# zhukovanadezhda/collaborative-filtering

Hardware: AMD Instinct MI355X
Metric: ratings/sec per ALS iteration at k=64 (higher is better)
Workload: dtype f32 (storage, solve, accumulate); Gram products as 2-way fp16 split (error <= 2^-23) on fp16 MFMA; rows over the condition limit redone in f64 (solve_dtype=auto)

## Files before the change

collaborative-filtering_amd/_hip.py:

```python
from __future__ import annotations

import ctypes as C
import os

_HERE = os.path.dirname(os.path.abspath(__file__))
LIB_PATH = os.environ.get("ALS_HIP_LIB") or os.path.join(_HERE, "csrc", "libals_hip.so")

SPLIT_CHUNK = 4096
MAX_K = 160

EXPORTS = ("als_version", "als_padded_k", "als_perm_index", "als_partial_slot_bytes", "als_partial_slot_bytes_f64",
           "als_row_solve", "als_factor_scale", "als_gs_sweep", "als_gs_sweep_levels", "als_gs_sweep_dataflow", "als_residual_stats", "als_w_normal_equations", "als_spd_solve_workspace_bytes", "als_spd_solve_f64", "als_item_stats", "als_item_stats_f64", "als_sum_pairs", "als_sumsq_partials",
           "als_sumsq", "als_history_row", "als_compose_z", "als_predict_at", "als_predict_dense",
           "als_topk_similarity", "als_graph_classify", "als_normalize_features", "als_impute_col_median",
           "als_host_coo_to_sides", "als_host_row_tasks", "als_host_level_schedule",
           "als_recommend_workspace_bytes", "als_recommend_topk", "als_rank_count_workspace_bytes", "als_rank_count",
           "als_recommend_topk_masked", "als_rank_count_masked",
           "als_fold_in", "als_fold_in_items", "als_explain", "als_mmr_rerank", "als_list_diversity")

_vp, _i32, _i64, _f32 = C.c_void_p, C.c_int32, C.c_int64, C.c_float


class RowSolveParams(C.Structure):
    _fields_ = [
        ("k", _i32), ("ld", _i32), ("nrows", _i64), ("F_zero_row", _i32), ("reserved0", _i32),
        ("gram_mode", _i32), ("ndual_tail", _i32), ("ndual_mid", _i32), ("F_scale_ready", _i32),
# ... 151 lines not shown
```

collaborative-filtering_amd/backend.py:

```python
from __future__ import annotations

import ctypes as C
import os
from typing import Optional

import torch

from . import _hip


def _p(t: Optional[torch.Tensor]):
    return None if t is None else C.c_void_p(t.data_ptr())


class HipBackend:
    name = "hip"

    GRAM_MODES = {"f32": 0, "f16x2": 1, "f64": 2}
    COND_LIMIT = 300.0
    PLANES_MAX_FLOATS = 16 << 20
    PLANES_MAX_FLOATS_K128 = (1 << 31) - 1

    def __init__(self, device: torch.device, gram: str = "f16x2", solve_dtype: str = "auto"):
        if gram not in ("f32", "f16x2"):
# ... 55 lines not shown
        p.sumr2_out, p.stat_out = _p(sumr2_out), _p(stat_out)
        p.tasks, p.ntasks = _p(tasks.tasks), tasks.ntasks
        p.ndual_tail = int(tasks.ndual)
        p.ndual_mid = int(tasks.nmid)
        p.long_rows, p.nlong = _p(tasks.long_rows), tasks.nlong
        p.workspace = _p(workspace)
        p.F_scale, p.F_scale_ready = _p(self._fscale), 0
        nwords = (int(zero_row) + 1) * ld
        limit = self.planes_max_floats if ld == 64 else (self.planes_max_floats_k128 if ld == 128 else 0)
        if (not f64 and p.gram_mode == self.GRAM_MODES["f16x2"] and 0 < nwords <= limit
                and int(zero_row) >= F.shape[0] - 1 and F.is_contiguous()):
            buf = self._planes.get(nwords)
            if buf is None:
                buf = self._planes[nwords] = torch.empty(nwords, dtype=torch.int32, device=self.device)
            p.F_planes = _p(buf)
        if self.cond_limit > 0.0 and not self.ablate and not f64:
            if side.nrows not in self._redo_rows:
                self._redo_rows[side.nrows] = torch.empty(max(side.nrows, 1), dtype=torch.int32, device=self.device)
            p.cond_limit = self.cond_limit
            p.redo_count, p.redo_rows = _p(self._redo_count), _p(self._redo_rows[side.nrows])
            p.cond_out = _p(self.cond_probe) if (self.cond_probe is not None and self.cond_probe.numel() >= side.nrows) else None
        self._check(self.lib.als_row_solve(C.byref(p), self._stream()), "als_row_solve")

    def gs_level(self, *, items, **kw):
        p = self._gs_params(items, kw)
        self._check(self.lib.als_gs_sweep(C.byref(p), self._stream()), "als_gs_sweep")

    def _gs_params(self, items, kw):
        p = _hip.GsSweepParams()
        p.k, p.ld = kw["k"], kw["ld"]
        p.items, p.nitems = _p(items), items.numel()
# ... 223 lines not shown
```

collaborative-filtering_amd/csrc/als_device.hpp:

```cpp
#pragma once
#include <hip/hip_runtime.h>
#include <stdint.h>
#include <type_traits>

typedef float f32x4 __attribute__((ext_vector_type(4)));
typedef float f32x2 __attribute__((ext_vector_type(2)));

#define ALS_EPS 1e-10f

#define ALS_KB_CASE_(N, ...) case N: { constexpr int KB = N; __VA_ARGS__; } break;
#define ALS_DISPATCH_KB(kb, ...)                                                                           \
    switch (kb) {                                                                                          \
        ALS_KB_CASE_(1, __VA_ARGS__) ALS_KB_CASE_(2, __VA_ARGS__) ALS_KB_CASE_(3, __VA_ARGS__)             \
        ALS_KB_CASE_(4, __VA_ARGS__) ALS_KB_CASE_(5, __VA_ARGS__) ALS_KB_CASE_(6, __VA_ARGS__)             \
        ALS_KB_CASE_(7, __VA_ARGS__) ALS_KB_CASE_(8, __VA_ARGS__) ALS_KB_CASE_(9, __VA_ARGS__)             \
        ALS_KB_CASE_(10, __VA_ARGS__)                                                                      \
        default: return ALS_E_BADK;                                                                        \
    }

__device__ __forceinline__ float readlane_f(float v, int src_lane) {
    return __int_as_float(__builtin_amdgcn_readlane(__float_as_int(v), src_lane));
}
__device__ __forceinline__ float bperm_f(float v, int src_lane) {
    return __int_as_float(__builtin_amdgcn_ds_bpermute(src_lane << 2, __float_as_int(v)));
}
__device__ __forceinline__ int bperm_i(int v, int src_lane) {
    return __builtin_amdgcn_ds_bpermute(src_lane << 2, v);
}
template <unsigned long long MASK>
__device__ __forceinline__ float select_lanes(float a, float b) {
    return __builtin_amdgcn_inverse_ballot_w64(MASK) ? a : b;
}
template <int BOUND, int RR>
constexpr unsigned long long lanes_below() {
    constexpr int n = BOUND - 64 * RR;
    return n <= 0 ? 0ull : (n >= 64 ? ~0ull : ((1ull << n) - 1ull));
}

__device__ __forceinline__ float wave_sum(float v) {
    auto dpp = [](float x, auto ctrl, auto rows) {
        return __int_as_float(__builtin_amdgcn_update_dpp(0, __float_as_int(x), decltype(ctrl)::value,
                                                          decltype(rows)::value, 0xf, false));
    };
    using std::integral_constant;
    v += dpp(v, integral_constant<int, 0xB1>{}, integral_constant<int, 0xf>{});
    v += dpp(v, integral_constant<int, 0x4E>{}, integral_constant<int, 0xf>{});
// ... 11 lines not shown
    uint32_t u = (uint32_t)__float_as_int(v);
    u = max(u, dpp(u, integral_constant<int, 0xB1>{}, integral_constant<int, 0xf>{}));
    u = max(u, dpp(u, integral_constant<int, 0x4E>{}, integral_constant<int, 0xf>{}));
    u = max(u, dpp(u, integral_constant<int, 0x141>{}, integral_constant<int, 0xf>{}));
    u = max(u, dpp(u, integral_constant<int, 0x140>{}, integral_constant<int, 0xf>{}));
    u = max(u, dpp(u, integral_constant<int, 0x142>{}, integral_constant<int, 0xa>{}));
    u = max(u, dpp(u, integral_constant<int, 0x143>{}, integral_constant<int, 0xc>{}));
    return __int_as_float(__builtin_amdgcn_readlane((int)u, 63));
}
__device__ __forceinline__ double wave_sum_d(double v) {
#pragma unroll
    for (int o = 32; o >= 1; o >>= 1) v += __shfl_xor(v, o, 64);
    return v;
}

__device__ __forceinline__ void wave_lds_sync() {
    __builtin_amdgcn_fence(__ATOMIC_SEQ_CST, "workgroup");
    __builtin_amdgcn_wave_barrier();
}

template <int KB>
__device__ __forceinline__ int perm_to_col(int p) { return KB * (p & 15) + (p >> 4); }

template <int KB>
__device__ __forceinline__ void load_frow(const float* __restrict__ p, float (&f)[KB]) {
    if constexpr (KB % 4 == 0) {
#pragma unroll
        for (int j = 0; j < KB / 4; ++j) {
            f32x4 v = *reinterpret_cast<const f32x4*>(p + 4 * j);
            f[4 * j] = v.x; f[4 * j + 1] = v.y; f[4 * j + 2] = v.z; f[4 * j + 3] = v.w;
        }
    } else if constexpr (KB % 2 == 0) {
// ... 400 lines not shown
```

collaborative-filtering_amd/csrc/row_common.hpp:

```cpp
#pragma once
#include <type_traits>
#include "als_device.hpp"

namespace {

__host__ __device__ constexpr int blk_idx(int I, int K) { return I * (I + 1) / 2 + K; }

typedef _Float16 h16x8 __attribute__((ext_vector_type(8)));
typedef _Float16 h16x2 __attribute__((ext_vector_type(2)));
typedef int i32x4 __attribute__((ext_vector_type(4)));

__device__ __forceinline__ void split2(float x0, float x1, float S, int& H, int& L) {
    const float y0 = x0 * S, y1 = x1 * S;
    const h16x2 h = __builtin_convertvector(f32x2{y0, y1}, h16x2);
    const float d0 = fmaf((float)h[0], -1.0f, y0), d1 = fmaf((float)h[1], -1.0f, y1);
    const h16x2 l = __builtin_convertvector(f32x2{d0, d1}, h16x2);
    H = __builtin_bit_cast(int, h);
    L = __builtin_bit_cast(int, l);
}

__device__ __forceinline__ void mfma_results_settle() {
    __builtin_amdgcn_sched_barrier(0);
    asm volatile("s_nop 15\n\ts_nop 3" ::: "memory");
    __builtin_amdgcn_sched_barrier(0);
}

template <int KB>
struct Chol {
    static constexpr int NR = KCfg<KB>::NR;
    float di[NR];
    float y[NR];
    float b[NR];
};

template <int KB>
__device__ __forceinline__ bool chol_spd(const Chol<KB>& S, int lane) {
    bool bad = false;
#pragma unroll
    for (int rr = 0; rr < KCfg<KB>::NR; ++rr) {
        const float v = S.di[rr];
        bad = bad || ((lane + 64 * rr < KCfg<KB>::KP) && !(v > 0.f && v < __builtin_inff()));
    }
    return __builtin_amdgcn_ballot_w64(bad) == 0;
}

template <int KB, int T2>
__device__ __forceinline__ void panel_trailing(float (&p)[KCfg<KB>::NR][16], const float (&l)[KCfg<KB>::NR], float lrep) {
    if constexpr (T2 < 16) {
#pragma unroll
        for (int rr = 0; rr < KCfg<KB>::NR; ++rr)
            asm("v_fmac_f32_dpp %0, %1, %2 row_newbcast:%3 row_mask:0xf bank_mask:0xf"
                : "+v"(p[rr][T2]) : "v"(lrep), "v"(l[rr]), "n"(T2));
        panel_trailing<KB, T2 + 1>(p, l, lrep);
    }
}

template <int KB, int RR, int T, int PB>
__device__ __forceinline__ void bwd_coeff_one(const float* __restrict__ Ls, const int (&colbase)[KCfg<KB>::NR][4],
                                              const Chol<KB>& S, float (&cf)[KCfg<KB>::NR][16]) {
    constexpr int prow = 16 * PB + T;
    const float v = Ls[colbase[RR][(T >> 2) & 3] + prow * 16];
    cf[RR][T] = select_lanes<lanes_below<prow, RR>()>(v * S.di[RR], 0.f);
    if constexpr (T + 1 < 16) bwd_coeff_one<KB, RR, T + 1, PB>(Ls, colbase, S, cf);
    else if constexpr (RR + 1 < KCfg<KB>::NR) bwd_coeff_one<KB, RR + 1, 0, PB>(Ls, colbase, S, cf);
}
template <int KB, int PB0>
__device__ __forceinline__ void bwd_coeffs(const float* __restrict__ Ls, const int (&colbase)[KCfg<KB>::NR][4],
                                           const Chol<KB>& S, float (&cf)[KCfg<KB>::NR][16],
                                           std::integral_constant<int, PB0>, int pb) {
    if (pb == PB0) bwd_coeff_one<KB, 0, 0, PB0>(Ls, colbase, S, cf);
    else if constexpr (PB0 + 1 < KB) bwd_coeffs<KB>(Ls, colbase, S, cf, std::integral_constant<int, PB0 + 1>{}, pb);
}

template <int KB>
__device__ __forceinline__ void backward_solve(const float* __restrict__ Ls, const Chol<KB>& S,
                                               float (&x)[KCfg<KB>::NR], int lane) {
    using C = KCfg<KB>;
// ... 31 lines not shown
```

collaborative-filtering_amd/csrc/row_solve.hip:

```cpp
#include <type_traits>
#include "als_device.hpp"
#include "als_hip.h"
#include "row_common.hpp"
#include "slot_fold.hpp"

namespace {

template <int KB>
struct RowAcc {
    f32x4 acc[KCfg<KB>::NACC];
    float rhs[KB];
    float cs[KB];
    float sumr;
    float sumr2;
    __device__ __forceinline__ void zero() {
#pragma unroll
        for (int a = 0; a < KCfg<KB>::NACC; ++a) acc[a] = f32x4{0.f, 0.f, 0.f, 0.f};
#pragma unroll
        for (int b = 0; b < KB; ++b) { rhs[b] = 0.f; cs[b] = 0.f; }
        sumr = 0.f; sumr2 = 0.f;
    }
};

template <int KB, bool FULL>
// ... 160 lines not shown
#pragma unroll
        for (int r = 0; r < 4; ++r) {
            Ls[(a * 4 + r) * 64 + lane] = A.acc[a][r];
            A.acc[a][r] = 0.f;
        }
}

template <int KB>
__device__ __forceinline__ void unflush_acc(RowAcc<KB>& A, const float* __restrict__ Ls, int lane) {
#pragma unroll
    for (int a = 0; a < KCfg<KB>::NACC; ++a)
#pragma unroll
        for (int r = 0; r < 4; ++r) A.acc[a][r] += Ls[(a * 4 + r) * 64 + lane];
}

template <int KB, int MODE>
__device__ __forceinline__ void gram_accumulate(RowAcc<KB>& A, const int32_t* __restrict__ idxp,
                                                const float* __restrict__ valp, int len,
                                                const float* __restrict__ F, int ld, int zero_row,
                                                const float* __restrict__ bias_other, float mu,
                                                float bself, int lane, float* __restrict__ Ls, float S,
                                                const uint32_t* __restrict__ planes = nullptr) {
    const int c = lane & 15, q = lane >> 4;
    const float* Fc = F + KB * c;
    int nflush = 0;
    f32x4 E[MODE == 2 ? KB : 1];
    const uint32_t* Pc = planes + KB * c;
    const int sel_c = (c == 0) ? 0x05040100 : (c == 2) ? 0x07060302 : 0x0c0c0c0c;
    const int ones_c = (c == 1) ? 0x3C003C00 : 0;
    const float inv_s = __int_as_float((254 - ((__float_as_int(S) >> 23) & 0xff)) << 23);
    if constexpr (MODE == 2) {
#pragma unroll
        for (int b = 0; b < KB; ++b) E[b] = f32x4{0.f, 0.f, 0.f, 0.f};
    }
    int idx1 = (lane < len) ? __builtin_nontemporal_load(idxp + lane) : zero_row;
    int idx2 = (64 + lane < len) ? __builtin_nontemporal_load(idxp + 64 + lane) : zero_row;
    float val1 = (lane < len) ? __builtin_nontemporal_load(valp + lane) : 0.f;
    float bo1 = (lane < len) ? bias_other[idx1] : 0.f;
    for (int base = 0; base < len; base += 64) {
        const int idx0 = idx1;
        const float val0 = val1, bo0 = bo1;
        idx1 = idx2;
        const int t2 = base + 128 + lane;
        idx2 = (t2 < len) ? __builtin_nontemporal_load(idxp + t2) : zero_row;
        const int t1 = base + 64 + lane;
        val1 = (t1 < len) ? __builtin_nontemporal_load(valp + t1) : 0.f;
        bo1 = (t1 < len) ? bias_other[idx1] : 0.f;
        const int nvalid = min(64, len - base);
        const bool ok = lane < nvalid;
        const float rb = val0 - mu - bo0;
        A.sumr += ok ? rb : 0.f;
        A.sumr2 = ok ? fmaf(rb, rb, A.sumr2) : A.sumr2;
        const float r0 = ok ? (rb - bself) : 0.f;
// ... 65 lines not shown
    constexpr int DR = (16 * J) >> 6, DL = (16 * J) & 63;
    const float prep = bperm_f(p[DR][T], DL + (lane & 15));
    const float d = readlane_f(p[RP][T], LP);
    const float inv = __builtin_amdgcn_rsqf(d);
    float l[NR];
#pragma unroll
    for (int rr = 0; rr < NR; ++rr) { l[rr] = p[rr][T] * inv; p[rr][T] = l[rr]; }
    float lrep = -(prep * inv);
    asm("s_nop 1" : "+v"(lrep));
    float yt = 0.f;
    if constexpr (SOLVE) yt = readlane_f(S.b[RP], LP) * inv;
    panel_trailing<KB, T + 1>(p, l, lrep);
    if constexpr (SOLVE) {
#pragma unroll
        for (int rr = 0; rr < NR; ++rr) S.b[rr] = fmaf(-l[rr], yt, S.b[rr]);
        S.y[RP] = select_lanes<1ull << LP>(yt, S.y[RP]);
    }
}

template <int KB, int J, int T, bool SOLVE>
__device__ __forceinline__ void panel_pivots(float (&p)[KCfg<KB>::NR][16], Chol<KB>& S, int lane) {
    if constexpr (T < 16) {
        panel_pivot<KB, J, T, SOLVE>(p, S, lane);
        panel_pivots<KB, J, T + 1, SOLVE>(p, S, lane);
    }
}

template <int KB, int J, bool SOLVE>
__device__ __forceinline__ void chol_panel(RowAcc<KB>& A, Chol<KB>& S, float* __restrict__ Ls, int lane) {
    using C = KCfg<KB>;
    constexpr int KP = C::KP, NR = C::NR;
    constexpr int OFF = C::lcol_off(J);
    const int c = lane & 15, q = lane >> 4;
    {
        const int swzc = (((c >> 2) ^ q) << 2) + (c & 3);
#pragma unroll
        for (int I = J; I < KB; ++I)
#pragma unroll
            for (int r = 0; r < 4; ++r)
                Ls[OFF + (16 * (I - J) + 4 * q + r) * 16 + swzc] = A.acc[blk_idx(I, J)][r];
    }
    wave_lds_sync();
    float p[NR][16];
    const int si = (lane >> 2) & 3;
#pragma unroll
    for (int rr = 0; rr < NR; ++rr) {
        const int i = lane + 64 * rr;
        const int rowi = min(max(i, 16 * J), KP - 1) - 16 * J;
#pragma unroll
        for (int g = 0; g < 4; ++g) {
            const f32x4 v = *reinterpret_cast<const f32x4*>(Ls + OFF + rowi * 16 + ((g ^ si) << 2));
            p[rr][4 * g] = v.x; p[rr][4 * g + 1] = v.y; p[rr][4 * g + 2] = v.z; p[rr][4 * g + 3] = v.w;
        }
    }
    wave_lds_sync();
    panel_pivots<KB, J, 0, SOLVE>(p, S, lane);
#pragma unroll
    for (int rr = 0; rr < NR; ++rr) {
        const int i = lane + 64 * rr;
        if (i >= 16 * J && i < KP) {
#pragma unroll
            for (int g = 0; g < 4; ++g) {
                const f32x4 v = {p[rr][4 * g], p[rr][4 * g + 1], p[rr][4 * g + 2], p[rr][4 * g + 3]};
                *reinterpret_cast<f32x4*>(Ls + OFF + (i - 16 * J) * 16 + ((g ^ si) << 2)) = v;
            }
        }
    }
    wave_lds_sync();
    {
        constexpr int DR = (16 * J) >> 6, DL = (16 * J) & 63;
        const float dl = Ls[OFF + c * 16 + (c & 3)];
        S.di[DR] = select_lanes<0xFFFFull << DL>(__builtin_amdgcn_rcpf(dl), S.di[DR]);
    }
    if constexpr (J + 1 < KB) {
        f32x4 op[KB - J - 1];
        const int sg = ((q ^ ((c >> 2) & 3)) << 2);
#pragma unroll
        for (int I = J + 1; I < KB; ++I)
            op[I - J - 1] = *reinterpret_cast<const f32x4*>(Ls + OFF + (16 * (I - J) + c) * 16 + sg);
#pragma unroll
        for (int K = J + 1; K < KB; ++K) {
            const f32x4 nb = -op[K - J - 1];
#pragma unroll
            for (int I = K; I < KB; ++I)
#pragma unroll
                for (int e = 0; e < 4; ++e)
                    A.acc[blk_idx(I, K)] = __builtin_amdgcn_mfma_f32_16x16x4f32(
                        op[I - J - 1][e], nb[e], A.acc[blk_idx(I, K)], 0, 0, 0);
        }
    }
}

template <int KB, int J, bool SOLVE>
__device__ __forceinline__ void chol_panels(RowAcc<KB>& A, Chol<KB>& S, float* __restrict__ Ls, int lane) {
    if constexpr (J < KB) {
        chol_panel<KB, J, SOLVE>(A, S, Ls, lane);
        chol_panels<KB, J + 1, SOLVE>(A, S, Ls, lane);
    }
}

template <int KB>
__device__ __forceinline__ bool row_needs_f64(const Chol<KB>& S, const als_row_solve_params& P, int row, bool spd,
                                              float mean_eig, float short_row_bound, int lane) {
    float dmx = 0.f, dmn = 0.f;
#pragma unroll
    for (int rr = 0; rr < KCfg<KB>::NR; ++rr) {
        const bool in = lane + 64 * rr < KCfg<KB>::KP;
        const float d = in ? S.di[rr] : 0.f;
        dmx = fmaxf(dmx, d);
        dmn = fmaxf(dmn, in ? __builtin_amdgcn_rcpf(d) : 0.f);
    }
    dmx = wave_max_nonneg(fmaxf(dmx, 0.f));
// ... 7 lines not shown
}

template <int KB>
__device__ __forceinline__ float gram_trace(const RowAcc<KB>& A, int lane) {
    const int c = lane & 15, q = lane >> 4;
    float t = 0.f;
#pragma unroll
    for (int J = 0; J < KB; ++J) {
        const f32x4 a = A.acc[blk_idx(J, J)];
        const float lo = (c & 1) ? a[1] : a[0], hi = (c & 1) ? a[3] : a[2];
        t += (c & 2) ? hi : lo;
    }
    return wave_sum((q == (c >> 2)) ? t : 0.f);
}

template <int KB>
__device__ __forceinline__ void finish_row(RowAcc<KB>& A, const als_row_solve_params& P, int row,
                                           float* __restrict__ Ls, int lane) {
    using C = KCfg<KB>;
    constexpr int KP = C::KP, NR = C::NR;
    const int c = lane & 15, q = lane >> 4;
    const int64_t r64 = row;

    if (P.gram_mode == ALS_GRAM_F16X2) {
        const float un = P.F_scale[1];
#pragma unroll
        for (int a = 0; a < C::NACC; ++a) A.acc[a] *= un;
    }

#pragma unroll
    for (int b = 0; b < KB; ++b) {
        A.rhs[b] += __shfl_xor(A.rhs[b], 16, 64); A.rhs[b] += __shfl_xor(A.rhs[b], 32, 64);
        A.cs[b] += __shfl_xor(A.cs[b], 16, 64);   A.cs[b] += __shfl_xor(A.cs[b], 32, 64);
    }
    const float sumr = wave_sum(A.sumr);
    const float sumr2 = wave_sum(A.sumr2);

    Chol<KB> S;
    float csrow[NR];
    int colrow[NR];
#pragma unroll
    for (int rr = 0; rr < NR; ++rr) {
        float bsel = 0.f, csel = 0.f;
#pragma unroll
        for (int e = 0; e < 4; ++e) {
            constexpr int dummy = 0; (void)dummy;
            const int b = (4 * rr + e < KB) ? 4 * rr + e : KB - 1;
            if (4 * rr + e < KB) {
                bsel = (q == e) ? A.rhs[b] : bsel;
                csel = (q == e) ? A.cs[b] : csel;
            }
        }
        S.b[rr] = bsel; S.di[rr] = 0.f; S.y[rr] = 0.f;
        csrow[rr] = csel;
        colrow[rr] = perm_to_col<KB>(min(lane + 64 * rr, KP - 1));
    }

    if (P.gram_out) {
        float* G = P.gram_out + r64 * KP * KP;
#pragma unroll
        for (int I = 0; I < KB; ++I)
#pragma unroll
            for (int K = 0; K <= I; ++K)
#pragma unroll
                for (int r = 0; r < 4; ++r)
                    G[(16 * I + 4 * q + r) * KP + 16 * K + c] = A.acc[blk_idx(I, K)][r];
    }
#pragma unroll
    for (int rr = 0; rr < NR; ++rr) {
        const int i = lane + 64 * rr;
        if (i < KP) {
            if (P.rhs_out) P.rhs_out[r64 * KP + i] = S.b[rr];
            if (P.colsum_out) P.colsum_out[r64 * KP + i] = csrow[rr];
        }
    }
    if (P.sumr_out && lane == 0) P.sumr_out[row] = sumr;
    if (P.sumr2_out && lane == 0) P.sumr2_out[row] = sumr2;

    const float lam = (P.lambda_row ? P.lambda_row[row] : P.lambda_scalar) + ALS_EPS
                    + (P.diag_extra ? P.diag_extra[row] : 0.f);
    float mean_eig = 0.f, short_row_bound = 0.f;
    if (P.cond_limit > 0.f) {
        const int64_t nrat = P.indptr[row + 1] - P.indptr[row];
        mean_eig = gram_trace<KB>(A, lane) / fmaxf((float)min((int64_t)P.k, nrat), 1.f) + lam;
        short_row_bound = (nrat < 4 * (int64_t)P.k) ? mean_eig / lam : 0.f;
    }
#pragma unroll
    for (int J = 0; J < KB; ++J) {
        const float dv = (perm_to_col<KB>(16 * J + c) < P.k) ? lam : 1.0f;
#pragma unroll
        for (int r = 0; r < 4; ++r) A.acc[blk_idx(J, J)][r] += (4 * q + r == c) ? dv : 0.f;
    }

    if (P.factor_out) {
        chol_panels<KB, 0, false>(A, S, Ls, lane);
        const bool spd = chol_spd<KB>(S, lane);
        if (P.cond_limit > 0.f) {
            if (row_needs_f64<KB>(S, P, row, spd, mean_eig, short_row_bound, lane)) return;
        } else if (!spd && lane == 0) atomicMax(P.status, row + 1);
        float* M = P.factor_out + r64 * KP * KP;
#pragma unroll
        for (int rr = 0; rr < NR; ++rr) {
            const int i = lane + 64 * rr;
            const int ic = min(i, KP - 1);
            const int colb = C::lcol_off_rt(ic >> 4) - 16 * (ic >> 4) * 16 + (c & 3);
#pragma unroll 8
            for (int p = 0; p < KP; ++p) {
                const int Jp = p >> 4;
                const int rowv = max(ic, 16 * Jp);
                const float lrow = Ls[C::lcol_off_rt(Jp) + (rowv - 16 * Jp) * 16 +
                                      ((((p >> 2) & 3) ^ ((rowv >> 2) & 3)) << 2) + (p & 3)];
                const int rsafe = max(p, ic & ~15);
                const float lcolv = Ls[colb + rsafe * 16 + (((c >> 2) ^ ((rsafe >> 2) & 3)) << 2)];
                if (i < KP) __builtin_nontemporal_store((p == i) ? S.di[rr] : (p < i ? lrow : lcolv), M + p * KP + i);
            }
        }
        return;
    }

    float rhs0[NR];
#pragma unroll
    for (int rr = 0; rr < NR; ++rr) rhs0[rr] = S.b[rr];
    if (P.rhs_extra) {
#pragma unroll
        for (int rr = 0; rr < NR; ++rr)
            if (lane + 64 * rr < KP) S.b[rr] += P.rhs_extra[r64 * P.ld + colrow[rr]];
    }
    if (!(P.reserved0 & 2)) {
        chol_panels<KB, 0, true>(A, S, Ls, lane);
        const bool spd = chol_spd<KB>(S, lane);
        if (P.cond_limit > 0.f) {
            if (row_needs_f64<KB>(S, P, row, spd, mean_eig, short_row_bound, lane)) return;
        } else if (!spd && lane == 0) atomicMax(P.status, row + 1);
    }
    float x[NR];
    if (!(P.reserved0 & 4)) backward_solve<KB>(Ls, S, x, lane);
    else {
#pragma unroll
        for (int rr = 0; rr < NR; ++rr) x[rr] = S.y[rr];
    }

    float dot = 0.f, xr = 0.f, yy = 0.f, xx = 0.f;
#pragma unroll
    for (int rr = 0; rr < NR; ++rr) {
        if (lane + 64 * rr < KP) {
            dot = fmaf(csrow[rr], x[rr], dot);
            xr = fmaf(rhs0[rr], x[rr], xr);
            yy = fmaf(S.y[rr], S.y[rr], yy);
            xx = fmaf(x[rr], x[rr], xx);
        }
    }
    dot = wave_sum(dot);
    const float nnz = (float)(P.indptr[row + 1] - P.indptr[row]);
    const float lb = P.lambda_bias_row ? P.lambda_bias_row[row] : P.lambda_bias_scalar;
    const float bnew = (sumr - dot) / (nnz + lb + ALS_EPS);
    const float bold = P.bias_self[row];
    float st1 = 0.f, st2 = 0.f;
    if (P.stat_out) {
        xr = wave_sum(xr); yy = wave_sum(yy); xx = wave_sum(xx);
        const double bn = bnew, dt = dot;
        const double s1 = (double)sumr - (double)nnz * bn;
        const double s2 = (double)sumr2 - 2.0 * bn * (double)sumr + (double)nnz * bn * bn;
        const double cross = (double)xr + ((double)bold - bn) * dt;
        const double quad = (double)yy - (double)lam * (double)xx;
        const double sd2 = s2 - 2.0 * cross + quad;
        if (P.cond_limit > 0.f && !(sd2 >= 1e-3 * s2)) {
            if (lane == 0) P.redo_rows[atomicAdd(P.redo_count, 1)] = row;
            return;
        }
        st1 = (float)(s1 - dt);
        st2 = (float)sd2;
    }
#pragma unroll
    for (int rr = 0; rr < NR; ++rr)
        if (lane + 64 * rr < KP) P.X_out[r64 * P.ld + colrow[rr]] = x[rr];
    __builtin_amdgcn_sched_barrier(0);
    if (lane == 0) {
        P.bias_out[row] = bnew;
        if (P.stat_out) { P.stat_out[2 * r64] = st1; P.stat_out[2 * r64 + 1] = st2; }
    }
}

template <int KB, int MODE>
__global__ __launch_bounds__(64 * KCfg<KB>::WPW, KCfg<KB>::MINW)
void k_row_tasks(const als_row_solve_params P) {
    using C = KCfg<KB>;
    __shared__ __attribute__((aligned(16))) float lds_all[C::WPW * C::LDS_FLOATS];
    const int lane = threadIdx.x & 63;
    const int wave = threadIdx.x >> 6;
    const int wave_u = wave;
    const int64_t tid = (int64_t)blockIdx.x * C::WPW + wave_u;
    if (tid >= P.ntasks) return;
    const als_task t = P.tasks[tid];
    const int row = t.row;
    const int seg = t.seg;
    const int slot = t.slot;
    const int64_t rbeg = P.indptr[row], rend = P.indptr[row + 1];
    const int64_t beg = rbeg + (int64_t)seg * ALS_SPLIT_CHUNK;
    const int len = (int)min((int64_t)ALS_SPLIT_CHUNK, rend - beg);
    const float mu = (float)(*P.mu);
    const float bself = P.bias_self[row];

    const float S = (MODE != 0) ? P.F_scale[0] : 1.f;

    RowAcc<KB> A;
    A.zero();
    if (!(P.reserved0 & 1))
        gram_accumulate<KB, MODE>(A, P.indices + beg, P.vals + beg, len, P.F, P.ld, P.F_zero_row,
                                  P.bias_other, mu, bself, lane, lds_all + wave * C::LDS_FLOATS, S,
                                  (const uint32_t*)P.F_planes);
    if (slot >= 0) {
        store_partial<KB>(A, (float*)P.workspace + (size_t)slot * C::SLOT_ITEMS * 64, lane);
        return;
    }
    finish_row<KB>(A, P, row, lds_all + wave_u * C::LDS_FLOATS, lane);
}

template <int KB, int NB>
__device__ __forceinline__ void row_dual(const als_row_solve_params& P, int row, int64_t beg, int len,
                                         float* __restrict__ Ls, int lane) {
    constexpr int KP = KCfg<KB>::KP, NR = KCfg<KB>::NR, NSLAB = (KP + 31) / 32;
    constexpr int NS = KCfg<NB>::NR;
    const int c = lane & 15, q = lane >> 4;
    const float bold = P.bias_self[row];
    const float mu = (float)*P.mu;
    bool ok[NS];
    int idx_l[NS];
    float r_l[NS];
#pragma unroll
    for (int ss = 0; ss < NS; ++ss) {
// ... 259 lines not shown
            h[2 * v4] = (uint32_t)h01; h[2 * v4 + 1] = (uint32_t)h23;
            l[2 * v4] = (uint32_t)l01; l[2 * v4 + 1] = (uint32_t)l23;
        }
        if constexpr (KB == 4) {
            reinterpret_cast<u32x4*>(planes)[e] = u32x4{h[0], h[1], l[0], l[1]};
        } else {
            reinterpret_cast<u32x4*>(planes)[2 * e] = u32x4{h[0], h[1], h[2], h[3]};
            reinterpret_cast<u32x4*>(planes)[2 * e + 1] = u32x4{l[0], l[1], l[2], l[3]};
        }
    }
}

template <int KB>
int launch_row_solve(const als_row_solve_params* p, hipStream_t st) {
    using C = KCfg<KB>;
    const bool plain = p->gram_mode == ALS_GRAM_F16X2 && p->reserved0 == 0 && p->X_out && p->bias_out &&
                       !p->gram_out && !p->factor_out && !p->rhs_out && !p->colsum_out && !p->sumr_out &&
                       !p->sumr2_out && !p->rhs_extra && !p->diag_extra;
    int64_t ntail = 0, nmid = 0;
    if (plain && p->ndual_tail >= 0 && p->ndual_mid >= 0 && (int64_t)p->ndual_tail + p->ndual_mid <= p->ntasks) {
        ntail = p->ndual_tail;
        if constexpr (KB >= 7) nmid = p->ndual_mid;
    }
    const int64_t nprimal = p->ntasks - ntail - nmid;
    if (nprimal > 0) {
        als_row_solve_params q = *p;
        q.ntasks = nprimal;
        const unsigned grid = (unsigned)((nprimal + C::WPW - 1) / C::WPW);
        bool planes = false;
        if constexpr (KB == 4 || KB == 8)
            planes = p->gram_mode == ALS_GRAM_F16X2 && p->F_planes != nullptr && p->reserved0 == 0;
        if (planes) {
            if constexpr (KB == 4 || KB == 8) {
                const int64_t npieces = ((int64_t)p->F_zero_row + 1) * 16;
                const unsigned sgrid = (unsigned)min((int64_t)4096, (npieces + 255) / 256);
                hipLaunchKernelGGL(k_split_planes<KB>, dim3(sgrid), dim3(256), 0, st, p->F, npieces, p->F_scale,
                                   (uint32_t*)p->F_planes);
                hipLaunchKernelGGL((k_row_tasks<KB, 2>), dim3(grid), dim3(64 * C::WPW), 0, st, q);
            }
        } else if (p->gram_mode == ALS_GRAM_F16X2)
            hipLaunchKernelGGL((k_row_tasks<KB, 1>), dim3(grid), dim3(64 * C::WPW), 0, st, q);
        else
            hipLaunchKernelGGL((k_row_tasks<KB, 0>), dim3(grid), dim3(64 * C::WPW), 0, st, q);
    }
    {
        if (ntail > 0)
            hipLaunchKernelGGL(k_row_dual<KB>, dim3((unsigned)((ntail + 3) / 4)), dim3(256), 0, st, *p, nprimal + nmid, ntail);
    }
    if constexpr (KB >= 7) {
        if (nmid > 0)
            hipLaunchKernelGGL(k_row_dual_mid<KB>, dim3((unsigned)((nmid + 1) / 2)), dim3(128), 0, st, *p, nprimal, nmid);
    }
    if (p->nlong > 0) {
        if (p->nlong * SumSlots<KB>::GROUPS > (int64_t)0x7FFFFFFF) return ALS_E_BADARG;
        hipLaunchKernelGGL(k_sum_slots<KB>, dim3((unsigned)(p->nlong * SumSlots<KB>::GROUPS)), dim3(64), 0, st,
                           p->long_rows, (float*)p->workspace);
        const unsigned grid = (unsigned)((p->nlong + C::WPW - 1) / C::WPW);
        hipLaunchKernelGGL(k_row_long<KB>, dim3(grid), dim3(64 * C::WPW), 0, st, *p);
    }
    return hipGetLastError() == hipSuccess ? 0 : ALS_E_LAUNCH;
}

}

int als_row_solve_f64_dispatch(const als_row_solve_params* p, hipStream_t st);
int als_row_redo_f64_dispatch(const als_row_solve_params* p, hipStream_t st);

extern "C" int als_version(void) { return ALS_HIP_VERSION; }
extern "C" int als_padded_k(int k) { return (k < 1 || k > ALS_MAX_K) ? ALS_E_BADK : 16 * ((k + 15) / 16); }
extern "C" int als_perm_index(int k, int c) {
    const int ld = als_padded_k(k);
    if (ld < 0 || c < 0 || c >= ld) return ALS_E_BADARG;
    const int KB = ld / 16;
    return 16 * (c % KB) + c / KB;
}
extern "C" int64_t als_partial_slot_bytes(int k) {
    const int ld = als_padded_k(k);
    if (ld < 0) return ALS_E_BADK;
    const int KB = ld / 16;
    return (int64_t)(KB * (KB + 1) / 2 * 4 + 2 * KB + 2) * 64 * sizeof(float);
}

extern "C" int als_factor_scale(const float* F, int64_t nfloats, float* scale, void* stream) {
// ... 45 lines not shown
```

include/als_hip.h:

```cpp
#ifndef ALS_HIP_H
#define ALS_HIP_H

#include <stddef.h>
#include <stdint.h>

#ifdef __cplusplus
extern "C" {
#endif

#define ALS_HIP_VERSION 103
#define ALS_NXCD 8

#define ALS_E_BADARG   (-1)
#define ALS_E_BADK     (-2)
#define ALS_E_LAUNCH   (-3)

#define ALS_GRAM_F32    0
#define ALS_GRAM_F16X2  1
#define ALS_GRAM_F64    2

#define ALS_MAX_K 160
#define ALS_SPLIT_CHUNK 4096

typedef struct als_task {
    int32_t row;
    int32_t seg;
    int32_t slot;
    int32_t reserved;
} als_task;

typedef struct als_long_row {
    int32_t row;
    int32_t slot0;
    int32_t nslots;
    int32_t reserved;
} als_long_row;

int als_version(void);
int als_padded_k(int k);
int als_perm_index(int k, int c);
int64_t als_partial_slot_bytes(int k);
int64_t als_partial_slot_bytes_f64(int k);

typedef struct als_row_solve_params {
    int32_t k;
    int32_t ld;
    int64_t nrows;
    int32_t F_zero_row;
    int32_t reserved0;
    int32_t gram_mode;
    int32_t ndual_tail;
    int32_t ndual_mid;
    int32_t F_scale_ready;
// ... 266 lines not shown
```

Baseline: 8.978 billion.

## Chain multiple row tasks per wave with prefetch of next row's head

For small K (KB<=4, so k=64), each wave now handles up to four row tasks in a grid-stride loop, with the grid sized in multiples of the XCD count. While the current row is being solved, the next row's task record, indptr, bias and first index/value chunk are prefetched, and the bias gather is issued in the middle of the Cholesky step. Task metadata is read through constant address space, and scalar-held lane masks replace some selects. The aim is to hide per-row load latency and launch/tail overhead, at the cost of fewer waves in flight and more register pressure.

```diff
diff --git a/collaborative-filtering_amd/_hip.py b/collaborative-filtering_amd/_hip.py
--- a/collaborative-filtering_amd/_hip.py
+++ b/collaborative-filtering_amd/_hip.py
@@ -9,7 +9,7 @@
 SPLIT_CHUNK = 4096
 MAX_K = 160
 
-EXPORTS = ("als_version", "als_padded_k", "als_perm_index", "als_partial_slot_bytes", "als_partial_slot_bytes_f64",
+EXPORTS = ("als_version", "als_rows_per_wave", "als_padded_k", "als_perm_index", "als_partial_slot_bytes", "als_partial_slot_bytes_f64",
            "als_row_solve", "als_factor_scale", "als_gs_sweep", "als_gs_sweep_levels", "als_gs_sweep_dataflow", "als_residual_stats", "als_w_normal_equations", "als_spd_solve_workspace_bytes", "als_spd_solve_f64", "als_item_stats", "als_item_stats_f64", "als_sum_pairs", "als_sumsq_partials",
            "als_sumsq", "als_history_row", "als_compose_z", "als_predict_at", "als_predict_dense",
            "als_topk_similarity", "als_graph_classify", "als_normalize_features", "als_impute_col_median",
diff --git a/collaborative-filtering_amd/backend.py b/collaborative-filtering_amd/backend.py
--- a/collaborative-filtering_amd/backend.py
+++ b/collaborative-filtering_amd/backend.py
@@ -93,7 +93,7 @@
             if buf is None:
                 buf = self._planes[nwords] = torch.empty(nwords, dtype=torch.int32, device=self.device)
             p.F_planes = _p(buf)
-        if self.cond_limit > 0.0 and not self.ablate and not f64:
+        if self.cond_limit > 0.0 and not (self.ablate & ~8) and not f64:
             if side.nrows not in self._redo_rows:
                 self._redo_rows[side.nrows] = torch.empty(max(side.nrows, 1), dtype=torch.int32, device=self.device)
             p.cond_limit = self.cond_limit
diff --git a/collaborative-filtering_amd/csrc/als_device.hpp b/collaborative-filtering_amd/csrc/als_device.hpp
--- a/collaborative-filtering_amd/csrc/als_device.hpp
+++ b/collaborative-filtering_amd/csrc/als_device.hpp
@@ -30,6 +30,10 @@
 template <unsigned long long MASK>
 __device__ __forceinline__ float select_lanes(float a, float b) {
     return __builtin_amdgcn_inverse_ballot_w64(MASK) ? a : b;
+}
+template <unsigned long long BASE, int SH>
+__device__ __forceinline__ float select_lanes_sh(float a, float b, int zero) {
+    return __builtin_amdgcn_inverse_ballot_w64(BASE << (SH + zero)) ? a : b;
 }
 template <int BOUND, int RR>
 constexpr unsigned long long lanes_below() {
@@ -71,8 +75,13 @@
     return v;
 }
 
+template <bool KEEP_LOADS = false>
 __device__ __forceinline__ void wave_lds_sync() {
-    __builtin_amdgcn_fence(__ATOMIC_SEQ_CST, "workgroup");
+    if constexpr (KEEP_LOADS) {
+        asm volatile("s_waitcnt lgkmcnt(0)" ::: "memory");
+    } else {
+        __builtin_amdgcn_fence(__ATOMIC_SEQ_CST, "workgroup");
+    }
     __builtin_amdgcn_wave_barrier();
 }
 
diff --git a/collaborative-filtering_amd/csrc/row_common.hpp b/collaborative-filtering_amd/csrc/row_common.hpp
--- a/collaborative-filtering_amd/csrc/row_common.hpp
+++ b/collaborative-filtering_amd/csrc/row_common.hpp
@@ -31,6 +31,7 @@
     float di[NR];
     float y[NR];
     float b[NR];
+    int zero = 0;
 };
 
 template <int KB>
@@ -60,7 +61,10 @@
                                               const Chol<KB>& S, float (&cf)[KCfg<KB>::NR][16]) {
     constexpr int prow = 16 * PB + T;
     const float v = Ls[colbase[RR][(T >> 2) & 3] + prow * 16];
-    cf[RR][T] = select_lanes<lanes_below<prow, RR>()>(v * S.di[RR], 0.f);
+    constexpr int nb = prow - 64 * RR;
+    if constexpr (nb <= 0) cf[RR][T] = 0.f;
+    else if constexpr (nb >= 64) cf[RR][T] = v * S.di[RR];
+    else cf[RR][T] = select_lanes_sh<~0ull, nb>(0.f, v * S.di[RR], S.zero);
     if constexpr (T + 1 < 16) bwd_coeff_one<KB, RR, T + 1, PB>(Ls, colbase, S, cf);
     else if constexpr (RR + 1 < KCfg<KB>::NR) bwd_coeff_one<KB, RR + 1, 0, PB>(Ls, colbase, S, cf);
 }
diff --git a/collaborative-filtering_amd/csrc/row_solve.hip b/collaborative-filtering_amd/csrc/row_solve.hip
--- a/collaborative-filtering_amd/csrc/row_solve.hip
+++ b/collaborative-filtering_amd/csrc/row_solve.hip
@@ -198,8 +198,45 @@
         for (int r = 0; r < 4; ++r) A.acc[a][r] += Ls[(a * 4 + r) * 64 + lane];
 }
 
+struct GramHead {
+    int idx1, idx2;
+    float val1, bo1;
+};
+
+__device__ __forceinline__ void gram_head_load(GramHead& h, const int32_t* __restrict__ idxp,
+                                               const float* __restrict__ valp, int len, int zero_row, int lane) {
+    h.idx1 = (lane < len) ? __builtin_nontemporal_load(idxp + lane) : zero_row;
+    h.idx2 = (64 + lane < len) ? __builtin_nontemporal_load(idxp + 64 + lane) : zero_row;
+    h.val1 = (lane < len) ? __builtin_nontemporal_load(valp + lane) : 0.f;
+}
+__device__ __forceinline__ void gram_head_bias(GramHead& h, int len, const float* __restrict__ bias_other, int lane) {
+    h.bo1 = (lane < len) ? bias_other[h.idx1] : 0.f;
+}
+
+struct HeadAhead {
+    int idx1, idx2;
+    float val1, bo1;
+};
+__device__ __forceinline__ void head_ahead_index(HeadAhead& a, const int32_t* __restrict__ idxp, int len, int lane) {
+    a.idx1 = __builtin_nontemporal_load(idxp + ((lane < len) ? lane : 0));
+}
+__device__ __forceinline__ void head_ahead_rest(HeadAhead& a, const int32_t* __restrict__ idxp,
+                                                const float* __restrict__ valp, int len,
+                                                const float* __restrict__ bias_other, int lane) {
+    a.bo1 = bias_other[a.idx1];
+    a.idx2 = __builtin_nontemporal_load(idxp + ((64 + lane < len) ? 64 + lane : 0));
+    a.val1 = __builtin_nontemporal_load(valp + ((lane < len) ? lane : 0));
+}
+__device__ __forceinline__ void head_from_ahead(GramHead& h, const HeadAhead& a, int len, int zero_row, int lane) {
+    const bool in1 = lane < len, in2 = 64 + lane < len;
+    h.idx1 = in1 ? a.idx1 : zero_row;
+    h.bo1 = in1 ? a.bo1 : 0.f;
+    h.idx2 = in2 ? a.idx2 : zero_row;
+    h.val1 = in1 ? a.val1 : 0.f;
+}
+
 template <int KB, int MODE>
-__device__ __forceinline__ void gram_accumulate(RowAcc<KB>& A, const int32_t* __restrict__ idxp,
+__device__ __forceinline__ void gram_accumulate(RowAcc<KB>& A, const GramHead& head, const int32_t* __restrict__ idxp,
                                                 const float* __restrict__ valp, int len,
                                                 const float* __restrict__ F, int ld, int zero_row,
                                                 const float* __restrict__ bias_other, float mu,
@@ -217,10 +254,8 @@
 #pragma unroll
         for (int b = 0; b < KB; ++b) E[b] = f32x4{0.f, 0.f, 0.f, 0.f};
     }
-    int idx1 = (lane < len) ? __builtin_nontemporal_load(idxp + lane) : zero_row;
-    int idx2 = (64 + lane < len) ? __builtin_nontemporal_load(idxp + 64 + lane) : zero_row;
-    float val1 = (lane < len) ? __builtin_nontemporal_load(valp + lane) : 0.f;
-    float bo1 = (lane < len) ? bias_other[idx1] : 0.f;
+    int idx1 = head.idx1, idx2 = head.idx2;
+    float val1 = head.val1, bo1 = head.bo1;
     for (int base = 0; base < len; base += 64) {
         const int idx0 = idx1;
         const float val0 = val1, bo0 = bo1;
@@ -316,7 +351,7 @@
     if constexpr (SOLVE) {
 #pragma unroll
         for (int rr = 0; rr < NR; ++rr) S.b[rr] = fmaf(-l[rr], yt, S.b[rr]);
-        S.y[RP] = select_lanes<1ull << LP>(yt, S.y[RP]);
+        S.y[RP] = select_lanes_sh<1ull, LP>(yt, S.y[RP], S.zero);
     }
 }
 
@@ -328,7 +363,7 @@
     }
 }
 
-template <int KB, int J, bool SOLVE>
+template <int KB, int J, bool SOLVE, bool KEEP = false>
 __device__ __forceinline__ void chol_panel(RowAcc<KB>& A, Chol<KB>& S, float* __restrict__ Ls, int lane) {
     using C = KCfg<KB>;
     constexpr int KP = C::KP, NR = C::NR;
@@ -342,7 +377,7 @@
             for (int r = 0; r < 4; ++r)
                 Ls[OFF + (16 * (I - J) + 4 * q + r) * 16 + swzc] = A.acc[blk_idx(I, J)][r];
     }
-    wave_lds_sync();
+    wave_lds_sync<KEEP>();
     float p[NR][16];
     const int si = (lane >> 2) & 3;
 #pragma unroll
@@ -355,7 +390,7 @@
             p[rr][4 * g] = v.x; p[rr][4 * g + 1] = v.y; p[rr][4 * g + 2] = v.z; p[rr][4 * g + 3] = v.w;
         }
     }
-    wave_lds_sync();
+    wave_lds_sync<KEEP>();
     panel_pivots<KB, J, 0, SOLVE>(p, S, lane);
 #pragma unroll
     for (int rr = 0; rr < NR; ++rr) {
@@ -368,11 +403,11 @@
             }
         }
     }
-    wave_lds_sync();
+    wave_lds_sync<KEEP>();
     {
         constexpr int DR = (16 * J) >> 6, DL = (16 * J) & 63;
         const float dl = Ls[OFF + c * 16 + (c & 3)];
-        S.di[DR] = select_lanes<0xFFFFull << DL>(__builtin_amdgcn_rcpf(dl), S.di[DR]);
+        S.di[DR] = select_lanes_sh<0xFFFFull, DL>(__builtin_amdgcn_rcpf(dl), S.di[DR], S.zero);
     }
     if constexpr (J + 1 < KB) {
         f32x4 op[KB - J - 1];
@@ -393,11 +428,11 @@
     }
 }
 
-template <int KB, int J, bool SOLVE>
+template <int KB, int J, bool SOLVE, bool KEEP = false>
 __device__ __forceinline__ void chol_panels(RowAcc<KB>& A, Chol<KB>& S, float* __restrict__ Ls, int lane) {
     if constexpr (J < KB) {
-        chol_panel<KB, J, SOLVE>(A, S, Ls, lane);
-        chol_panels<KB, J + 1, SOLVE>(A, S, Ls, lane);
+        chol_panel<KB, J, SOLVE, KEEP>(A, S, Ls, lane);
+        chol_panels<KB, J + 1, SOLVE, KEEP>(A, S, Ls, lane);
     }
 }
 
@@ -435,29 +470,46 @@
     return wave_sum((q == (c >> 2)) ? t : 0.f);
 }
 
-template <int KB>
+#define ALS_CONSTANT __attribute__((address_space(4)))
+template <class T>
+__device__ __forceinline__ const T ALS_CONSTANT* as_constant(const T* p) { return (const T ALS_CONSTANT*)p; }
+
+struct NoMid { __device__ __forceinline__ void operator()() const {} };
+struct ChainRow {
+    int nrat, row_u;
+    float bold, un;
+};
+
+template <int KB, class Mid = NoMid, bool CHAIN = false>
 __device__ __forceinline__ void finish_row(RowAcc<KB>& A, const als_row_solve_params& P, int row,
-                                           float* __restrict__ Ls, int lane) {
+                                           float* __restrict__ Ls, int lane, Mid mid = Mid{},
+                                           const ChainRow ch = ChainRow{}) {
     using C = KCfg<KB>;
     constexpr int KP = C::KP, NR = C::NR;
     const int c = lane & 15, q = lane >> 4;
     const int64_t r64 = row;
 
     if (P.gram_mode == ALS_GRAM_F16X2) {
-        const float un = P.F_scale[1];
+        const float un = CHAIN ? ch.un : P.F_scale[1];
 #pragma unroll
         for (int a = 0; a < C::NACC; ++a) A.acc[a] *= un;
     }
 
 #pragma unroll
     for (int b = 0; b < KB; ++b) {
-        A.rhs[b] += __shfl_xor(A.rhs[b], 16, 64); A.rhs[b] += __shfl_xor(A.rhs[b], 32, 64);
-        A.cs[b] += __shfl_xor(A.cs[b], 16, 64);   A.cs[b] += __shfl_xor(A.cs[b], 32, 64);
+        if constexpr (CHAIN) {
+            A.rhs[b] += bperm_f(A.rhs[b], lane ^ 16); A.rhs[b] += bperm_f(A.rhs[b], lane ^ 32);
+            A.cs[b] += bperm_f(A.cs[b], lane ^ 16);   A.cs[b] += bperm_f(A.cs[b], lane ^ 32);
+        } else {
+            A.rhs[b] += __shfl_xor(A.rhs[b], 16, 64); A.rhs[b] += __shfl_xor(A.rhs[b], 32, 64);
+            A.cs[b] += __shfl_xor(A.cs[b], 16, 64);   A.cs[b] += __shfl_xor(A.cs[b], 32, 64);
+        }
     }
     const float sumr = wave_sum(A.sumr);
     const float sumr2 = wave_sum(A.sumr2);
 
     Chol<KB> S;
+    if constexpr (CHAIN) asm volatile("s_mov_b32 %0, 0" : "=s"(S.zero));
     float csrow[NR];
     int colrow[NR];
 #pragma unroll
@@ -477,7 +529,7 @@
         colrow[rr] = perm_to_col<KB>(min(lane + 64 * rr, KP - 1));
     }
 
-    if (P.gram_out) {
+    if (!CHAIN && P.gram_out) {
         float* G = P.gram_out + r64 * KP * KP;
 #pragma unroll
         for (int I = 0; I < KB; ++I)
@@ -490,19 +542,19 @@
 #pragma unroll
     for (int rr = 0; rr < NR; ++rr) {
         const int i = lane + 64 * rr;
-        if (i < KP) {
+        if (!CHAIN && i < KP) {
             if (P.rhs_out) P.rhs_out[r64 * KP + i] = S.b[rr];
             if (P.colsum_out) P.colsum_out[r64 * KP + i] = csrow[rr];
         }
     }
-    if (P.sumr_out && lane == 0) P.sumr_out[row] = sumr;
-    if (P.sumr2_out && lane == 0) P.sumr2_out[row] = sumr2;
-
-    const float lam = (P.lambda_row ? P.lambda_row[row] : P.lambda_scalar) + ALS_EPS
-                    + (P.diag_extra ? P.diag_extra[row] : 0.f);
+    if (!CHAIN && P.sumr_out && lane == 0) P.sumr_out[row] = sumr;
+    if (!CHAIN && P.sumr2_out && lane == 0) P.sumr2_out[row] = sumr2;
+
+    const float lam = (P.lambda_row ? (CHAIN ? as_constant(P.lambda_row)[ch.row_u] : P.lambda_row[row]) : P.lambda_scalar)
+                    + ALS_EPS + ((!CHAIN && P.diag_extra) ? P.diag_extra[row] : 0.f);
     float mean_eig = 0.f, short_row_bound = 0.f;
     if (P.cond_limit > 0.f) {
-        const int64_t nrat = P.indptr[row + 1] - P.indptr[row];
+        const int64_t nrat = CHAIN ? (int64_t)ch.nrat : P.indptr[row + 1] - P.indptr[row];
         mean_eig = gram_trace<KB>(A, lane) / fmaxf((float)min((int64_t)P.k, nrat), 1.f) + lam;
         short_row_bound = (nrat < 4 * (int64_t)P.k) ? mean_eig / lam : 0.f;
     }
@@ -513,7 +565,7 @@
         for (int r = 0; r < 4; ++r) A.acc[blk_idx(J, J)][r] += (4 * q + r == c) ? dv : 0.f;
     }
 
-    if (P.factor_out) {
+    if (!CHAIN && P.factor_out) {
         chol_panels<KB, 0, false>(A, S, Ls, lane);
         const bool spd = chol_spd<KB>(S, lane);
         if (P.cond_limit > 0.f) {
@@ -542,20 +594,21 @@
     float rhs0[NR];
 #pragma unroll
     for (int rr = 0; rr < NR; ++rr) rhs0[rr] = S.b[rr];
-    if (P.rhs_extra) {
+    if (!CHAIN && P.rhs_extra) {
 #pragma unroll
         for (int rr = 0; rr < NR; ++rr)
             if (lane + 64 * rr < KP) S.b[rr] += P.rhs_extra[r64 * P.ld + colrow[rr]];
     }
-    if (!(P.reserved0 & 2)) {
-        chol_panels<KB, 0, true>(A, S, Ls, lane);
+    if (CHAIN || !(P.reserved0 & 2)) {
+        chol_panels<KB, 0, true, CHAIN>(A, S, Ls, lane);
+        mid();
         const bool spd = chol_spd<KB>(S, lane);
         if (P.cond_limit > 0.f) {
             if (row_needs_f64<KB>(S, P, row, spd, mean_eig, short_row_bound, lane)) return;
         } else if (!spd && lane == 0) atomicMax(P.status, row + 1);
     }
     float x[NR];
-    if (!(P.reserved0 & 4)) backward_solve<KB>(Ls, S, x, lane);
+    if (CHAIN || !(P.reserved0 & 4)) backward_solve<KB>(Ls, S, x, lane);
     else {
 #pragma unroll
         for (int rr = 0; rr < NR; ++rr) x[rr] = S.y[rr];
@@ -572,10 +625,11 @@
         }
     }
     dot = wave_sum(dot);
-    const float nnz = (float)(P.indptr[row + 1] - P.indptr[row]);
-    const float lb = P.lambda_bias_row ? P.lambda_bias_row[row] : P.lambda_bias_scalar;
+    const float nnz = CHAIN ? (float)(int64_t)ch.nrat : (float)(P.indptr[row + 1] - P.indptr[row]);
+    const float lb = P.lambda_bias_row ? (CHAIN ? as_constant(P.lambda_bias_row)[ch.row_u] : P.lambda_bias_row[row])
+                                       : P.lambda_bias_scalar;
     const float bnew = (sumr - dot) / (nnz + lb + ALS_EPS);
-    const float bold = P.bias_self[row];
+    const float bold = CHAIN ? ch.bold : P.bias_self[row];
     float st1 = 0.f, st2 = 0.f;
     if (P.stat_out) {
         xr = wave_sum(xr); yy = wave_sum(yy); xx = wave_sum(xx);
@@ -602,39 +656,137 @@
     }
 }
 
-template <int KB, int MODE>
+#ifndef ALS_ROWS_PER_WAVE
+#define ALS_ROWS_PER_WAVE 4
+#endif
+#ifndef ALS_ROW_AHEAD
+#define ALS_ROW_AHEAD 1
+#endif
+#define ALS_ABLATE_ONE_TASK 8
+
+struct TaskRow {
+    int row, slot, len;
+    int64_t beg;
+    float bself;
+};
+__device__ __forceinline__ als_task load_task(const als_task* tasks, int64_t i) {
+    const int32_t ALS_CONSTANT* w = as_constant(reinterpret_cast<const int32_t*>(tasks + i));
+    als_task t;
+    t.row = w[0]; t.seg = w[1]; t.slot = w[2]; t.reserved = 0;
+    return t;
+}
+__device__ __forceinline__ TaskRow task_row(const als_task t, const int64_t ALS_CONSTANT* indptr,
+                                            const float ALS_CONSTANT* bias_self) {
+    TaskRow r;
+    r.row = t.row; r.slot = t.slot;
+    const int64_t rend = indptr[t.row + 1];
+    r.beg = indptr[t.row] + (int64_t)t.seg * ALS_SPLIT_CHUNK;
+    r.len = (int)min((int64_t)ALS_SPLIT_CHUNK, rend - r.beg);
+    r.bself = bias_self[t.row];
+    return r;
+}
+
+template <int KB, int MODE, int R>
 __global__ __launch_bounds__(64 * KCfg<KB>::WPW, KCfg<KB>::MINW)
 void k_row_tasks(const als_row_solve_params P) {
     using C = KCfg<KB>;
     __shared__ __attribute__((aligned(16))) float lds_all[C::WPW * C::LDS_FLOATS];
     const int lane = threadIdx.x & 63;
     const int wave = threadIdx.x >> 6;
-    const int wave_u = wave;
+    const int wave_u = (R == 1) ? wave : __builtin_amdgcn_readfirstlane(wave);
     const int64_t tid = (int64_t)blockIdx.x * C::WPW + wave_u;
     if (tid >= P.ntasks) return;
-    const als_task t = P.tasks[tid];
-    const int row = t.row;
-    const int seg = t.seg;
-    const int slot = t.slot;
-    const int64_t rbeg = P.indptr[row], rend = P.indptr[row + 1];
-    const int64_t beg = rbeg + (int64_t)seg * ALS_SPLIT_CHUNK;
-    const int len = (int)min((int64_t)ALS_SPLIT_CHUNK, rend - beg);
-    const float mu = (float)(*P.mu);
-    const float bself = P.bias_self[row];
-
-    const float S = (MODE != 0) ? P.F_scale[0] : 1.f;
-
-    RowAcc<KB> A;
-    A.zero();
-    if (!(P.reserved0 & 1))
-        gram_accumulate<KB, MODE>(A, P.indices + beg, P.vals + beg, len, P.F, P.ld, P.F_zero_row,
-                                  P.bias_other, mu, bself, lane, lds_all + wave * C::LDS_FLOATS, S,
-                                  (const uint32_t*)P.F_planes);
-    if (slot >= 0) {
-        store_partial<KB>(A, (float*)P.workspace + (size_t)slot * C::SLOT_ITEMS * 64, lane);
-        return;
-    }
-    finish_row<KB>(A, P, row, lds_all + wave_u * C::LDS_FLOATS, lane);
+    if constexpr (R == 1) {
+        const als_task t = P.tasks[tid];
+        const int row = t.row;
+        const int seg = t.seg;
+        const int slot = t.slot;
+        const int64_t rbeg = P.indptr[row], rend = P.indptr[row + 1];
+        const int64_t beg = rbeg + (int64_t)seg * ALS_SPLIT_CHUNK;
+        const int len = (int)min((int64_t)ALS_SPLIT_CHUNK, rend - beg);
+        const float mu = (float)(*P.mu);
+        const float bself = P.bias_self[row];
+        const float S = (MODE != 0) ? P.F_scale[0] : 1.f;
+        RowAcc<KB> A;
+        A.zero();
+        if (!(P.reserved0 & 1)) {
+            GramHead h;
+            gram_head_load(h, P.indices + beg, P.vals + beg, len, P.F_zero_row, lane);
+            gram_head_bias(h, len, P.bias_other, lane);
+            gram_accumulate<KB, MODE>(A, h, P.indices + beg, P.vals + beg, len, P.F, P.ld, P.F_zero_row,
+                                      P.bias_other, mu, bself, lane, lds_all + wave * C::LDS_FLOATS, S,
+                                      (const uint32_t*)P.F_planes);
+        }
+        if (slot >= 0) {
+            store_partial<KB>(A, (float*)P.workspace + (size_t)slot * C::SLOT_ITEMS * 64, lane);
+            return;
+        }
+        finish_row<KB>(A, P, row, lds_all + wave_u * C::LDS_FLOATS, lane);
+    } else {
+        const int64_t G = (int64_t)gridDim.x * C::WPW;
+        float* Ls = lds_all + wave_u * C::LDS_FLOATS;
+        const float mu = (float)(*P.mu);
+        const float S = (MODE != 0) ? P.F_scale[0] : 1.f;
+        const float un = (MODE != 0) ? P.F_scale[1] : 1.f;
+        const int64_t ALS_CONSTANT* indptr = as_constant(P.indptr);
+        const float ALS_CONSTANT* bias_self = as_constant(P.bias_self);
+        als_task rec = load_task(P.tasks, tid);
+        als_task rec_next = (tid + G < P.ntasks) ? load_task(P.tasks, tid + G) : rec;
+        TaskRow t = task_row(rec, indptr, bias_self);
+        GramHead h;
+        gram_head_load(h, P.indices + t.beg, P.vals + t.beg, t.len, P.F_zero_row, lane);
+        gram_head_bias(h, t.len, P.bias_other, lane);
+#pragma unroll 1
+        for (int j = 0; j < R; ++j) {
+            const int64_t tid_next = tid + (int64_t)(j + 1) * G;
+            const bool more = j + 1 < R && tid_next < P.ntasks;
+            TaskRow tn = t;
+            als_task rec_after = rec_next;
+            if (more) {
+                tn = task_row(rec_next, indptr, bias_self);
+                if (j + 2 < R && tid_next + G < P.ntasks) rec_after = load_task(P.tasks, tid_next + G);
+            }
+            __builtin_amdgcn_sched_barrier(0);
+            int ln = lane;
+            asm volatile("" : "+v"(ln));
+            int len_v = t.len, beg_lo = (int)t.beg, beg_hi = (int)(t.beg >> 32);
+            asm volatile("" : "+v"(len_v), "+v"(beg_lo), "+v"(beg_hi));
+            const int64_t beg_v = (int64_t)(((uint64_t)(uint32_t)beg_hi << 32) | (uint32_t)beg_lo);
+            RowAcc<KB> A;
+            A.zero();
+            gram_accumulate<KB, MODE>(A, h, P.indices + beg_v, P.vals + beg_v, len_v, P.F, P.ld, P.F_zero_row,
+                                      P.bias_other, mu, t.bself, ln, Ls, S, (const uint32_t*)P.F_planes);
+            asm volatile("" : "+v"(ln));
+            HeadAhead ahead = {0, 0, 0.f, 0.f};
+            const bool pre = ALS_ROW_AHEAD && more && tn.len > 0;
+            if (pre) head_ahead_index(ahead, P.indices + tn.beg, tn.len, ln);
+            __builtin_amdgcn_sched_barrier(0);
+            const auto bias_ahead = [&]() {
+                __builtin_amdgcn_sched_barrier(0);
+                if (pre) head_ahead_rest(ahead, P.indices + tn.beg, P.vals + tn.beg, tn.len, P.bias_other, ln);
+                __builtin_amdgcn_sched_barrier(0);
+            };
+            int row_v = t.row, nrat_v = t.len;
+            asm volatile("" : "+v"(row_v), "+v"(nrat_v));
+            if (t.slot >= 0) {
+                store_partial<KB>(A, (float*)P.workspace + (size_t)t.slot * C::SLOT_ITEMS * 64, ln);
+                bias_ahead();
+            } else {
+                finish_row<KB, decltype(bias_ahead), true>(A, P, row_v, Ls, ln, bias_ahead,
+                                                           ChainRow{nrat_v, t.row, t.bself, un});
+            }
+            if (!more) break;
+            wave_lds_sync<true>();
+            t = tn;
+            rec_next = rec_after;
+            if (ALS_ROW_AHEAD) {
+                head_from_ahead(h, ahead, t.len, P.F_zero_row, ln);
+            } else {
+                gram_head_load(h, P.indices + t.beg, P.vals + t.beg, t.len, P.F_zero_row, ln);
+                gram_head_bias(h, t.len, P.bias_other, ln);
+            }
+        }
+    }
 }
 
 template <int KB, int NB>
@@ -924,7 +1076,8 @@
 template <int KB>
 int launch_row_solve(const als_row_solve_params* p, hipStream_t st) {
     using C = KCfg<KB>;
-    const bool plain = p->gram_mode == ALS_GRAM_F16X2 && p->reserved0 == 0 && p->X_out && p->bias_out &&
+    const int ablate = p->reserved0 & ~ALS_ABLATE_ONE_TASK;
+    const bool plain = p->gram_mode == ALS_GRAM_F16X2 && ablate == 0 && p->X_out && p->bias_out &&
                        !p->gram_out && !p->factor_out && !p->rhs_out && !p->colsum_out && !p->sumr_out &&
                        !p->sumr2_out && !p->rhs_extra && !p->diag_extra;
     int64_t ntail = 0, nmid = 0;
@@ -936,22 +1089,32 @@
     if (nprimal > 0) {
         als_row_solve_params q = *p;
         q.ntasks = nprimal;
-        const unsigned grid = (unsigned)((nprimal + C::WPW - 1) / C::WPW);
+        unsigned grid = (unsigned)((nprimal + C::WPW - 1) / C::WPW);
+        constexpr int R = (KB <= 4) ? ALS_ROWS_PER_WAVE : 1;
+        const bool chain = R > 1 && plain && !(p->reserved0 & ALS_ABLATE_ONE_TASK);
+        if (chain) {
+            constexpr int64_t unit = (int64_t)ALS_NXCD * C::WPW;
+            const int64_t G = ((nprimal + R - 1) / R + unit - 1) / unit * unit;
+            grid = (unsigned)(G / C::WPW);
+        }
         bool planes = false;
         if constexpr (KB == 4 || KB == 8)
-            planes = p->gram_mode == ALS_GRAM_F16X2 && p->F_planes != nullptr && p->reserved0 == 0;
+            planes = p->gram_mode == ALS_GRAM_F16X2 && p->F_planes != nullptr && ablate == 0;
+        const dim3 block(64 * C::WPW);
         if (planes) {
             if constexpr (KB == 4 || KB == 8) {
                 const int64_t npieces = ((int64_t)p->F_zero_row + 1) * 16;
                 const unsigned sgrid = (unsigned)min((int64_t)4096, (npieces + 255) / 256);
                 hipLaunchKernelGGL(k_split_planes<KB>, dim3(sgrid), dim3(256), 0, st, p->F, npieces, p->F_scale,
                                    (uint32_t*)p->F_planes);
-                hipLaunchKernelGGL((k_row_tasks<KB, 2>), dim3(grid), dim3(64 * C::WPW), 0, st, q);
-            }
-        } else if (p->gram_mode == ALS_GRAM_F16X2)
-            hipLaunchKernelGGL((k_row_tasks<KB, 1>), dim3(grid), dim3(64 * C::WPW), 0, st, q);
-        else
-            hipLaunchKernelGGL((k_row_tasks<KB, 0>), dim3(grid), dim3(64 * C::WPW), 0, st, q);
+                if (chain) hipLaunchKernelGGL((k_row_tasks<KB, 2, R>), dim3(grid), block, 0, st, q);
+                else hipLaunchKernelGGL((k_row_tasks<KB, 2, 1>), dim3(grid), block, 0, st, q);
+            }
+        } else if (p->gram_mode == ALS_GRAM_F16X2) {
+            if (chain) hipLaunchKernelGGL((k_row_tasks<KB, 1, R>), dim3(grid), block, 0, st, q);
+            else hipLaunchKernelGGL((k_row_tasks<KB, 1, 1>), dim3(grid), block, 0, st, q);
+        } else
+            hipLaunchKernelGGL((k_row_tasks<KB, 0, 1>), dim3(grid), block, 0, st, q);
     }
     {
         if (ntail > 0)
@@ -977,6 +1140,7 @@
 int als_row_redo_f64_dispatch(const als_row_solve_params* p, hipStream_t st);
 
 extern "C" int als_version(void) { return ALS_HIP_VERSION; }
+extern "C" int als_rows_per_wave(void) { return ALS_ROWS_PER_WAVE; }
 extern "C" int als_padded_k(int k) { return (k < 1 || k > ALS_MAX_K) ? ALS_E_BADK : 16 * ((k + 15) / 16); }
 extern "C" int als_perm_index(int k, int c) {
     const int ld = als_padded_k(k);
diff --git a/include/als_hip.h b/include/als_hip.h
--- a/include/als_hip.h
+++ b/include/als_hip.h
@@ -37,6 +37,7 @@
 } als_long_row;
 
 int als_version(void);
+int als_rows_per_wave(void);
 int als_padded_k(int k);
 int als_perm_index(int k, int c);
 int64_t als_partial_slot_bytes(int k);
```

New measurement: 8.966 billion. No clear change (-0.1%).
